# fudan-zvg/PARTNER

Hardware: AMD Instinct MI355X
Metric: frames/sec polar voxelize+PFN+BEV+head, 30k-pt sweep (whole job) (higher is better)
Workload: dtype f32

## Files before the change

include/partner_hip.h:

```cpp
#ifndef PARTNER_HIP_H
#define PARTNER_HIP_H

#include <stddef.h>
#include <stdint.h>

#ifdef __cplusplus
extern "C" {
#endif

#define PN_OK 0
#define PN_ERR_INVALID (-1)
#define PN_ERR_LAUNCH (-2)
#define PN_ERR_WORKSPACE (-3)

#define PN_ACT_NONE 0
#define PN_ACT_RELU 1
#define PN_ACT_TANH 2
#define PN_ACT_GELU 3

typedef void *pn_stream_t;

int pn_version(void);
int pn_last_error(char *buf, size_t buf_len);
int pn_device_count(void);
// ... 472 lines not shown
                               void *workspace, size_t workspace_bytes, pn_stream_t stream);
typedef struct {
  const float *src;
  int32_t pixel_stride;
  int32_t rows;
} pn_row_piece;
int pn_assemble_rows_f32(const pn_row_piece *pieces, int n_out, int out_rows, int w, int c, float *out,
                         int out_pixel_stride, int out_channel_offset, pn_stream_t stream);

int pn_nchw_to_nhwc_f32(const float *in, int b, int c, int h, int w, float *out, pn_stream_t stream);
int pn_nhwc_to_nchw_f32(const float *in, int b, int c, int h, int w, int pixel_stride,
                        int channel_offset, float *out, pn_stream_t stream);
int pn_transpose_hw_f32(const float *in, int b, int h, int w, int c, float *out, pn_stream_t stream);

typedef struct {
  pn_conv_desc desc;
  const float *in;
  const float *packed_w;
  const float *scale;
  const float *shift;
  float *out;
  float *stat_partials;
  int32_t stat_strata;
  int32_t stat_channel_groups;
  const float *stat_gamma;
  const float *stat_beta;
  float stat_eps;
  int32_t stat_affine_strata;
  float *stat_affine;
  float *stat_mean_rstd;
  const float *norm_affine;
  int32_t norm_strata;
  int32_t norm_channels;
} pn_conv_job;
size_t pn_conv_wino_packed_weight_floats(int cout, int cin);
int pn_pack_conv_weight_wino_f32(const float *w_oihw, int cout, int cin, float *packed, pn_stream_t stream);
int pn_pack_conv_dgrad_weight_wino_f32(const float *w_fwd_oihw, int cout_fwd, int cin_fwd, float *packed, pn_stream_t stream);
int pn_conv2d_wino_nhwc_f32(const pn_conv_desc *desc, const float *in, const float *packed_w, const float *scale,
                            const float *shift, float *out, pn_stream_t stream);
size_t pn_conv_wino4_packed_weight_floats(int cout, int cin);
int pn_pack_conv_weight_wino4_f32(const float *w_oihw, int cout, int cin, float *packed, pn_stream_t stream);
int pn_pack_conv_dgrad_weight_wino4_f32(const float *w_fwd_oihw, int cout_fwd, int cin_fwd, float *packed, pn_stream_t stream);
int pn_conv_wino4_tiles(const pn_conv_desc *desc);
int pn_conv2d_wino4_nhwc_f32(const pn_conv_desc *desc, const float *in, const float *packed_w, const float *scale,
                             const float *shift, float *out, pn_stream_t stream);
size_t pn_wino4_planes_floats(int batch, int h, int w, int c);
int pn_wino4_planes_from_nhwc_f32(const float *in, int batch, int h, int w, int c, int in_pixel_stride, int in_channel_offset,
                                  int transpose_hw, float *planes, pn_stream_t stream);
int pn_conv_wino4_chain_supported(const pn_conv_desc *desc);
int pn_conv2d_wino4_chain_f32(const pn_conv_desc *desc, const float *planes_in, const float *packed_w, const float *scale,
                              const float *shift, float *planes_out, float *out_nhwc, pn_stream_t stream);
size_t pn_conv_wino24_packed_weight_floats(int cout, int cin);
int pn_pack_conv_weight_wino24_f32(const float *w_oihw, int cout, int cin, float *packed, pn_stream_t stream);
int pn_conv_wino24_chain_supported(const pn_conv_desc *desc);
int pn_conv2d_wino24_chain_f32(const pn_conv_desc *desc, const float *planes_in, const float *packed_w24, const float *scale,
                               const float *shift, float *planes_out, float *out_nhwc, pn_stream_t stream);

size_t pn_conv_wino44_packed_weight_floats(int cout, int cin);
int pn_pack_conv_weight_wino44_f32(const float *w_oihw, int cout, int cin, float *packed, pn_stream_t stream);
int pn_conv_wino44_chain_supported(const pn_conv_desc *desc);
int pn_conv2d_wino44_chain_f32(const pn_conv_desc *desc, const float *planes_in, const float *packed_w44, const float *scale,
                               const float *shift, float *planes_out, float *out_nhwc, pn_stream_t stream);
typedef struct pn_head_stat_job {
  const float *partials;
  int32_t cout_total;
  int32_t channel_offset;
// ... 121 lines not shown
```

partner_amd/csrc/conv_mfma.hip:

```cpp
#include "pn_common.h"
#include "wino_planes.h"
#include <algorithm>
#include <cstdlib>

namespace {

using f32x16 = __attribute__((ext_vector_type(16))) float;
using f32x4 = __attribute__((ext_vector_type(4))) float;
using bf16x8 = __attribute__((ext_vector_type(8))) __bf16;

enum { DT_F32 = 0, DT_BF16 = 1, DT_BF16_F32OUT = 2 };

__device__ __forceinline__ unsigned short f32_to_bf16_rne(float f) {
  unsigned u = __builtin_bit_cast(unsigned, f);
  u += 0x7fffu + ((u >> 16) & 1u);
  return (unsigned short)(u >> 16);
}

enum { MODE_CONV = 0, MODE_DECONV2 = 1, MODE_STRAT = 2 };

struct ConvArgs {
  const float* in;
  const float* w;
  const float* scale;
// ... 539 lines not shown
          rpix = ((size_t)b * (2 * a.OH) + 2 * oh + (col_d[j] >> 1)) * (2 * a.OW) + 2 * ow + (col_d[j] & 1);
          dst = a.out + rpix * a.out_ps + col_off[j];
        }
        float o;
        if (a.res && a.res_pre_act) {
          o = pn::apply_act(fmaf(acc[i][j][r], sc[j], sh[j]) + a.res[rpix * a.res_ps + col_off[j]], a.act);
        } else {
          o = pn::apply_act(fmaf(acc[i][j][r], sc[j], sh[j]), a.act);
          if (a.res) o += a.res[rpix * a.res_ps + col_off[j]];
        }
        if constexpr (DT == DT_BF16)
          reinterpret_cast<unsigned short*>(a.out)[dst - a.out] = f32_to_bf16_rne(o);
        else
          *dst = o;
      }
    }
  }
}


template <int WM, int WN, int TM, int TN, int DT = DT_F32, bool GATHER = false, bool NORM_IN = false>
__global__ __launch_bounds__(WM* WN * 64) void conv_mfma_kernel(ConvArgs a) {
  constexpr int BN = WN * TN * 32;
  int bid = blockIdx.x;
  if constexpr (!GATHER) {
    const int nmt = a.nmt, q = nmt >> 3, r = nmt & 7, x = bid & 7, idx = bid >> 3;
    bid = (x < r ? x * (q + 1) : r * (q + 1) + (x - r) * q) + idx;
  }
  conv_body<WM, WN, TM, TN, DT, GATHER, NORM_IN>(a, bid, blockIdx.y * BN, blockIdx.z);
}

constexpr int kMaxJobs = 8;
struct MultiArgs {
  int njobs, total;
  int first[kMaxJobs + 1];
  ConvArgs job[kMaxJobs];
};

template <int WM, int WN, int TM, int TN, bool NORM_IN>
__global__ __launch_bounds__(WM* WN * 64) void conv_multi_kernel(MultiArgs m_by_value) {
  constexpr int BN = WN * TN * 32;
  typedef const __attribute__((address_space(4))) int* kptr_t;
  const kptr_t base = (kptr_t)__builtin_amdgcn_kernarg_segment_ptr();
  const int njobs = base[offsetof(MultiArgs, njobs) / 4], nt = base[offsetof(MultiArgs, total) / 4];
  const int bid = blockIdx.x;
  const int q = nt >> 3, r = nt & 7, x = bid & 7, idx = bid >> 3;
  const int t = (x < r ? x * (q + 1) : r * (q + 1) + (x - r) * q) + idx;
  int j = 0;
  for (int k = 1; k < njobs; ++k)
    if (t >= base[offsetof(MultiArgs, first) / 4 + k]) j = k;
  j = __builtin_amdgcn_readfirstlane(j);
  const int local = t - base[offsetof(MultiArgs, first) / 4 + j];
  static_assert(sizeof(ConvArgs) % 4 == 0 && offsetof(MultiArgs, job) % 4 == 0, "job table must be dword aligned");
  constexpr int JW = sizeof(ConvArgs) / 4;
  union { ConvArgs a; int w[JW]; } u;
  const kptr_t src = base + offsetof(MultiArgs, job) / 4 + j * JW;
#pragma unroll
  for (int i = 0; i < JW; ++i) u.w[i] = src[i];
  const ConvArgs& a = u.a;
  const int ntn = (a.ncols + BN - 1) / BN, per_z = a.nmt * ntn;
  const int z = local / per_z, rem = local - z * per_z;
  const int ny = rem / a.nmt, mt = rem - ny * a.nmt;
  conv_body<WM, WN, TM, TN, DT_F32, false, NORM_IN>(a, mt, ny * BN, z);
}


struct FinArgs {
  int njobs, total;
  int first[kMaxJobs + 1];
  int bm, wn;
  ConvArgs job[kMaxJobs];
};

__device__ __forceinline__ void group_geometry(const ConvArgs& a, int& pix_b, int& wsub, int& spr) {
  pix_b = a.OH * a.OWsub;
  wsub = a.OWsub / a.st_S;
  spr = a.st_S > 1 ? wsub / 32 : 1;
}

template <int NT>
__device__ __forceinline__ void fold_allch_group(const ConvArgs& a, const float2* part, int wn_count, int z, int b, int s, double* red,
                                                 double& o1, double& o2) {
  int pix_b, wsub, spr;
  group_geometry(a, pix_b, wsub, spr);
  const int tid = threadIdx.x;
// ... 1046 lines not shown
__global__ void f32_to_bf16_kernel(const float* __restrict__ x, unsigned short* __restrict__ y, size_t n) {
  for (size_t i = blockIdx.x * (size_t)blockDim.x + threadIdx.x; i < n; i += (size_t)gridDim.x * blockDim.x) y[i] = f32_to_bf16_rne(x[i]);
}

__global__ void bf16_to_f32_kernel(const unsigned short* __restrict__ x, float* __restrict__ y, size_t n) {
  for (size_t i = blockIdx.x * (size_t)blockDim.x + threadIdx.x; i < n; i += (size_t)gridDim.x * blockDim.x)
    y[i] = __builtin_bit_cast(float, (unsigned)x[i] << 16);
}

template <int WM, int WN, int TM, int TN, bool NORM_IN>
int launch_multi(MultiArgs& m, size_t extra_smem, hipStream_t st) {
  constexpr int BM = WM * TM * 32, BN = WN * TN * 32;
  constexpr size_t base = 2 * (size_t)(BM * A_LD + BK * BN) * sizeof(float);
  const size_t smem = base + extra_smem;
  PN_REQUIRE(smem <= 160 * 1024, "conv_multi: the normalisation table does not fit LDS");
  static size_t attr_smem[64] = {0};
  int dev = 0;
  (void)hipGetDevice(&dev);
  if (dev < 0 || dev >= 64 || attr_smem[dev] < smem) {
    (void)hipFuncSetAttribute(reinterpret_cast<const void*>(&conv_multi_kernel<WM, WN, TM, TN, NORM_IN>),
                              hipFuncAttributeMaxDynamicSharedMemorySize, (int)smem);
    if (dev >= 0 && dev < 64) attr_smem[dev] = smem;
  }
  int total = 0;
  for (int j = 0; j < m.njobs; ++j) {
    ConvArgs& a = m.job[j];
    a.nmt = pn::cdiv(a.M, BM);
    const int tiles_z = a.nmt * pn::cdiv(a.ncols, BN);
    m.first[j] = total;
    total += tiles_z * a.zdim;
  }
  m.first[m.njobs] = total;
  m.total = total;
  pn::ProfileSlot ps;
  if (pn::take_profile_slot(ps))
    hipExtLaunchKernelGGL((conv_multi_kernel<WM, WN, TM, TN, NORM_IN>), dim3(total), dim3(WM * WN * 64), smem, st, ps.start, ps.stop, 0, m);
  else
    hipLaunchKernelGGL((conv_multi_kernel<WM, WN, TM, TN, NORM_IN>), dim3(total), dim3(WM * WN * 64), smem, st, m);
  return pn::check_launch("conv_multi_kernel");
}

int tile_bm(int tile) { return tile == 1 ? 128 : 64; }

}

extern "C" {

}

namespace {

template <int K>
__device__ __forceinline__ float quad_bcast(float v) {
  return __builtin_bit_cast(float, __builtin_amdgcn_update_dpp(0, __builtin_bit_cast(int, v), K * 0x55, 0xf, 0xf, true));
}

template <int CIN>
__global__ __launch_bounds__(256) void sparse_conv_c16_kernel(const float* __restrict__ in, unsigned in_bytes, const int32_t* __restrict__ nbr,
                                                              const int32_t* __restrict__ n_out, int cap, int taps, const float* __restrict__ packed_w,
                                                              int quads, int cout_pad, const float* __restrict__ scale, const float* __restrict__ shift,
                                                              int act, const float* __restrict__ residual, float* __restrict__ out) {
  __shared__ __attribute__((aligned(16))) float wl[27 * 256];
  __shared__ int nb_s[64 * 27];
  const int tid = threadIdx.x, q = tid & 3, sl = tid >> 2;
  for (int i = tid; i < taps * 256; i += 256) {
    const int t = i >> 8, ci = (i >> 4) & 15, co = i & 15;
    wl[i] = ci < CIN ? packed_w[(((size_t)t * quads + (ci >> 2)) * cout_pad + co) * 4 + (ci & 3)] : 0.f;
  }
  const int n = min(*n_out, cap);
  const __amdgpu_buffer_rsrc_t rsrc = __builtin_amdgcn_make_buffer_rsrc(const_cast<float*>(in), 0, in_bytes, 0x00020000);
  const f32x4 sc = scale ? *reinterpret_cast<const f32x4*>(scale + 4 * q) : f32x4{1.f, 1.f, 1.f, 1.f};
  const f32x4 sh = shift ? *reinterpret_cast<const f32x4*>(shift + 4 * q) : f32x4{0.f, 0.f, 0.f, 0.f};
  for (int g = blockIdx.x; g * 64 < n; g += gridDim.x) {
    __syncthreads();
    for (int i = tid; i < 64 * taps; i += 256) nb_s[i] = g * 64 + i / taps < n ? nbr[(size_t)g * 64 * taps + i] : -1;
// ... 213 lines not shown
                              pn_stream_t stream) {
  PN_REQUIRE(pn_conv2d_nhwc_planes_supported(d), "conv_planes: not covered (groups 1, cout % 8 == 0, output rows of 4 .. 64 pixels dividing 64, or of 128)");
  PN_REQUIRE(in && packed_w && planes && ((uintptr_t)in & 15) == 0 && ((uintptr_t)packed_w & 15) == 0 && ((uintptr_t)planes & 15) == 0 &&
                 ((uintptr_t)scale & 15) == 0 && ((uintptr_t)shift & 15) == 0, "conv_planes: null or misaligned pointer");
  ConvArgs a;
  int zdim = 1;
  if (int rc = fill_args(d, a, zdim)) return rc;
  a.in = in; a.w = packed_w; a.scale = scale; a.shift = shift;
  a.out = planes; a.out_ps = d->cout; a.out_co = 0;
  a.planes = planes;
  a.plane_floats = (unsigned)((size_t)d->batch * (a.OH + 2) * (a.OW / 4) * 4);
  hipStream_t st = pn::S(stream);
  if (a.OW == 128) {
    const long long t128 = (long long)pn::cdiv(a.M, 128) * pn::cdiv(a.ncols, 128);
    return t128 >= 384 ? launch_conv<2, 2, 2, 2>(a, zdim, st) : launch_conv<4, 2, 1, 1>(a, zdim, st);
  }
  return dispatch_conv(a, zdim, st);
}

size_t pn_conv_stat_partial_floats(const pn_conv_desc* d, int tile) {
  ConvArgs a;
  int zdim = 1;
  if (fill_args(d, a, zdim)) return 0;
  const int bm = tile_bm(tile);
  return (size_t)zdim * pn::cdiv(a.M, bm) * (bm / 32) * a.cout_pad * 2;
}

static int tile_wn(int tile) { return tile == 5 ? 4 : (tile == 4 ? 1 : 2); }

static int job_to_args(const pn_conv_job& jb, int tile, ConvArgs& a, size_t& extra) {
  int zdim = 1;
  if (int rc = fill_args(&jb.desc, a, zdim)) return rc;
  const pn_conv_desc* d = &jb.desc;
  PN_REQUIRE(jb.in && jb.packed_w && jb.out, "conv_multi: null pointer");
  PN_REQUIRE(d->cin % 4 == 0 && d->in_pixel_stride % 4 == 0 && d->in_channel_offset % 4 == 0,
             "conv_multi: cin, input pixel stride and channel offset must be multiples of 4");
  PN_REQUIRE(((uintptr_t)jb.in & 15) == 0 && ((uintptr_t)jb.packed_w & 15) == 0, "conv_multi: pointers must be 16-byte aligned");
  PN_REQUIRE(!d->accumulate, "conv_multi: accumulate is not supported");
  a.in = jb.in; a.w = jb.packed_w; a.scale = jb.scale; a.shift = jb.shift; a.out = jb.out;
  a.zdim = zdim;
  const int bm = tile_bm(tile), bn = tile_wn(tile) * (tile == 1 ? 64 : 32);
  a.nmt = pn::cdiv(a.M, bm);
  a.st_segs_z = a.nmt * (bm / 32);
  if (jb.stat_partials) {
    PN_REQUIRE(a.mode != MODE_DECONV2, "conv_multi: no statistics for the transposed convolution");
    PN_REQUIRE((a.Cout % 4 == 0) && (a.out_ps % 4 == 0) && (a.out_co % 4 == 0) && (((uintptr_t)a.out & 15) == 0),
               "conv_multi: statistics need the vectorised epilogue (channel counts / offsets multiples of 4)");
    PN_REQUIRE(a.mode == MODE_STRAT || zdim == 1, "conv_multi: statistics of grouped convolutions are not supported");
    PN_REQUIRE(a.ncols <= bn, "conv_multi: statistics need the job's columns in one column tile");
    const int S = jb.stat_strata < 1 ? 1 : jb.stat_strata;
    PN_REQUIRE(S == 1 || (a.mode == MODE_CONV && a.OWsub % S == 0 && (a.OWsub / S) % 32 == 0),
               "conv_multi: stat_strata needs a plain convolution whose strata are multiples of 32 columns");
    PN_REQUIRE(a.B == 1 || (a.OH * a.OWsub) % (jb.stat_channel_groups > 1 ? bm : 32) == 0,
               "conv_multi: with batch > 1 a sample must be a whole number of tiles (per-channel statistics) / 32-row segments");
    PN_REQUIRE(jb.stat_channel_groups == 1 || jb.stat_channel_groups == a.ncols, "conv_multi: channel groups must be 1 or the column count");
    const int slots = a.mode == MODE_STRAT ? zdim : S;
    PN_REQUIRE(jb.stat_affine_strata >= slots, "conv_multi: stat_affine_strata too small");
    a.st_part = jb.stat_partials; a.st_S = S; a.st_cg = jb.stat_channel_groups;
    a.st_gamma = jb.stat_gamma; a.st_beta = jb.stat_beta; a.st_eps = jb.stat_eps;
    a.st_ab = jb.stat_affine; a.st_ab_S = jb.stat_affine_strata; a.st_stat = jb.stat_mean_rstd;
  }
  if (jb.norm_affine) {
    PN_REQUIRE(jb.norm_strata >= 1 && a.W % jb.norm_strata == 0 && a.KW <= 3 && a.KH * a.KW <= 16, "conv_multi: bad normalise-on-load geometry");
    PN_REQUIRE(jb.norm_channels >= a.Cin * (d->groups > 1 ? d->groups : 1) && a.B * jb.norm_strata < 1024, "conv_multi: normalisation table too small / too many groups");
    a.ni_ab = jb.norm_affine; a.ni_S = jb.norm_strata; a.ni_C = jb.norm_channels;
    extra = std::max(extra, (size_t)a.B * a.ni_S * a.ni_C * 2 * sizeof(float));
  }
  return PN_OK;
}

int pn_conv2d_multi_f32(const pn_conv_job* jobs, int njobs, int tile, pn_stream_t stream) {
  PN_REQUIRE(jobs && njobs >= 1 && njobs <= kMaxJobs, "conv_multi: 1 .. 8 jobs");
  PN_REQUIRE(tile == 1 || tile == 3 || tile == 4 || tile == 5, "conv_multi: tile must be 1 (128x128), 3 (64x64), 4 (64x32) or 5 (64x128)");
  MultiArgs m;
  memset(&m, 0, sizeof(m));
  m.njobs = njobs;
  bool norm_in = false;
  size_t extra = 0;
  for (int j = 0; j < njobs; ++j) {
    if (int rc = job_to_args(jobs[j], tile, m.job[j], extra)) return rc;
    norm_in = norm_in || m.job[j].ni_ab != nullptr;
  }
  if (norm_in)
    for (int j = 0; j < njobs; ++j) PN_REQUIRE(m.job[j].ni_ab, "conv_multi: normalise-on-load must be given for every job of the launch or for none");
  hipStream_t st = pn::S(stream);
  switch (tile) {
    case 1: PN_REQUIRE(!norm_in, "conv_multi: tile 1 has no normalise-on-load variant"); return launch_multi<2, 2, 2, 2, false>(m, 0, st);
    case 3: return norm_in ? launch_multi<2, 2, 1, 1, true>(m, extra, st) : launch_multi<2, 2, 1, 1, false>(m, 0, st);
    case 4: return norm_in ? launch_multi<2, 1, 1, 1, true>(m, extra, st) : launch_multi<2, 1, 1, 1, false>(m, 0, st);
    default: PN_REQUIRE(!norm_in, "conv_multi: tile 5 has no normalise-on-load variant"); return launch_multi<2, 4, 1, 1, false>(m, 0, st);
  }
}

int pn_conv3x3_tap_sum_f32(const float* g, int ldg, int batch, int h, int w, int cout, const float* scale, const float* shift, int act, float* out,
                           int out_pixel_stride, int out_channel_offset, pn_stream_t stream) {
  PN_REQUIRE(g && out && batch >= 1 && h >= 1 && w >= 1 && cout >= 1 && cout <= 3 && ldg >= 9 * cout, "conv3x3_tap_sum: bad arguments (cout 1 .. 3, ldg >= 9 cout)");
  PN_REQUIRE(out_pixel_stride >= out_channel_offset + cout && out_channel_offset >= 0, "conv3x3_tap_sum: channel slice does not fit the pixel stride");
  PN_REQUIRE((long long)batch * h * w * cout < (1ll << 31), "conv3x3_tap_sum: map too large");
  const int total = batch * h * w * cout;
  hipLaunchKernelGGL(conv_tap_sum_kernel, dim3(pn::cdiv(total, 256)), dim3(256), 0, pn::S(stream), g, ldg, batch, h, w, cout, scale, shift, act, out,
                     out_pixel_stride, out_channel_offset);
  return pn::check_launch("conv_tap_sum_kernel");
}

int pn_conv2d_small_n_multi_f32(const pn_conv_job* jobs, int njobs, pn_stream_t stream) {
  PN_REQUIRE(jobs && njobs >= 1 && njobs <= kMaxJobs, "conv_small_n_multi: 1 .. 8 jobs");
  MultiArgs m;
  memset(&m, 0, sizeof(m));
  m.njobs = njobs;
  int total = 0;
  int order[kMaxJobs], no = 0;
  for (int pass = 0; pass < 2; ++pass)
    for (int j = 0; j < njobs; ++j)
      if ((jobs[j].desc.kh * jobs[j].desc.kw == 9) == (pass == 0)) order[no++] = j;
  for (int jo = 0; jo < njobs; ++jo) {
    const int j = jo;
    ConvArgs& a = m.job[j];
    size_t extra = 0;
    if (int rc = job_to_args(jobs[order[jo]], 3, a, extra)) return rc;
    const int taps = a.KH * a.KW;
    PN_REQUIRE(a.mode == MODE_CONV && a.zdim == 1 && a.ncols <= 12 && a.Cin <= 64 && (taps == 9 || taps == 1) && !jobs[order[jo]].stat_partials,
               "conv_small_n_multi: plain 1x1 / 3x3 convolutions with <= 64 input channels and <= 12 output columns, no statistics");
// ... 110 lines not shown
```

partner_amd/hip.py:

```python
from __future__ import annotations

import ctypes as C
import os
from typing import Optional

import torch

_LIB_PATH = os.path.join(os.path.dirname(os.path.abspath(__file__)), "lib", "libpartner_hip.so")
_lib: Optional[C.CDLL] = None

ACT_NONE, ACT_RELU, ACT_TANH, ACT_GELU = 0, 1, 2, 3


class PartnerHipError(RuntimeError):
    pass


class ConvDesc(C.Structure):

    _fields_ = [(n, C.c_int32) for n in (
        "batch", "in_h", "in_w", "cin", "cout", "groups", "kh", "kw", "stride", "pad_h", "pad_w",
        "in_pixel_stride", "in_channel_offset", "out_pixel_stride", "out_channel_offset", "act", "deconv2x2",
        "range_strata", "pad_h_end", "pad_w_end", "accumulate", "frames_in_flight", "transpose_hw")]


class RowPiece(C.Structure):

    _fields_ = [("src", C.c_void_p), ("pixel_stride", C.c_int32), ("rows", C.c_int32)]


class HeadStatJob(C.Structure):

    _fields_ = [("partials", C.c_void_p), ("cout_total", C.c_int32), ("channel_offset", C.c_int32), ("channels", C.c_int32), ("strata", C.c_int32),
                ("gamma", C.c_void_p), ("beta", C.c_void_p), ("eps", C.c_float), ("table", C.c_void_p)]


class ChainHeadJob(C.Structure):

    _fields_ = [("desc", C.POINTER(ConvDesc)), ("planes_in", C.c_void_p), ("packed_w24", C.c_void_p), ("scale", C.c_void_p), ("shift", C.c_void_p),
                ("planes_out", C.c_void_p), ("out_nhwc", C.c_void_p), ("stat_partials", C.c_void_p)]


class ConvJob(C.Structure):

    _fields_ = [("desc", ConvDesc), ("in_", C.c_void_p), ("packed_w", C.c_void_p), ("scale", C.c_void_p), ("shift", C.c_void_p),
                ("out", C.c_void_p), ("stat_partials", C.c_void_p), ("stat_strata", C.c_int32),
                ("stat_channel_groups", C.c_int32), ("stat_gamma", C.c_void_p), ("stat_beta", C.c_void_p), ("stat_eps", C.c_float),
                ("stat_affine_strata", C.c_int32), ("stat_affine", C.c_void_p), ("stat_mean_rstd", C.c_void_p),
                ("norm_affine", C.c_void_p), ("norm_strata", C.c_int32), ("norm_channels", C.c_int32)]


_P = C.c_void_p
_I = C.c_int
_F = C.c_float
_SZ = C.c_size_t
_U64 = C.c_uint64

SIGNATURES = {
    "pn_version": (_I, []),
    "pn_last_error": (_I, [C.c_char_p, _SZ]),
    "pn_device_count": (_I, []),
    "pn_cart_to_polar_f32": (_I, [_P, _I, _I, _P, _P]),
    "pn_polar_grid_index_f32": (_I, [_P, _I, _I, _P, _I, _P, _P, _P, _P, _P, _P]),
    "pn_keys_from_grid_ind": (_I, [_P, _I, _P, _I, _P, _P]),
    "pn_unique_workspace_bytes": (_SZ, [_U64, _I]),
    "pn_unique_rank_bitmap": (_I, [_P, _I, _P, _U64, _P, _P, _P, _P, _P, _P, _SZ, _P]),
    "pn_unique_keys_ptr": (_P, [_P, _U64, _I]),
    "pn_bucket_workspace_bytes": (_SZ, [_I]),
    "pn_bucket_points": (_I, [_P, _P, _I, _P, _P, _P, _P, _P, _SZ, _P]),
    "pn_voxel_index_fused_state_bytes": (_SZ, [_U64]),
    "pn_voxel_index_fused_f32": (_I, [_P, _I, _I, _P, _I, _P, _P, _P, _P, _P, _P, _P, _P, _SZ, _P, _P, _P, _P, _P]),
    "pn_voxel_index_fused_rows_f32": (_I, [_P, _I, _I, _P, _I, _P, _P, _P, _P, _P, _P, _P, _P, _SZ, _P, _P, _P, _P, _P, _P]),
    "pn_voxel_index_fused_sweeps_f32": (_I, [_P, _I, _I, _P, _I, _P, _P, _F, _P, _P, _P, _P, _P, _P, _P, _P, _SZ, _P, _P, _P, _P, _P, _P]),
    "pn_clear_frame_cells": (_I, [_P, _P, _I, _P, _I, _P, _P, _P]),
    "pn_sort_voxel_runs": (_I, [_P, _P, _I, _P, _P, _P]),
    "pn_hard_voxelize_workspace_bytes": (_SZ, [_U64, _I, _I]),
    "pn_hard_voxelize_f32": (_I, [_P, _I, _I, _I, _P, _P, _I, _I, _P, _P, _P, _P, _P, _SZ, _P]),
    "pn_scatter_mean_f32": (_I, [_P, _I, _I, _P, _P, _P, _I, _P, _P]),
    "pn_hard_voxel_mean_f32": (_I, [_P, _P, _I, _I, _I, _P, _P]),
    "pn_concat_voxel_segments_f32": (_I, [_P, _P, _P, _I, _I, _I, _P, _P, _P, _P]),
    "pn_dynamic_pfn_fwd": (_I, [_P, _I, _P, _P, _P, _I, _P, _P, _P, _I, _P, _I, _F, _F, _F, _F, _P, _P, _P]),
    "pn_pfn_center_table_floats": (_SZ, [_I]),
# ... 283 lines not shown
```

partner_amd/necks.py:

```python
from __future__ import annotations

import logging

import numpy as np
import torch
from torch import nn

from . import hip, ops
from .builder import NECKS
from .nn_utils import PlanCache, Sequential, build_norm_layer, eval_only


@NECKS.register_module
class RPN(nn.Module):
    def __init__(self, layer_nums, ds_layer_strides, ds_num_filters, us_layer_strides, us_num_filters,
                 num_input_features, norm_cfg=None, name="rpn", logger=None, **kwargs):
        super().__init__()
        self._layer_strides = ds_layer_strides
        self._num_filters = ds_num_filters
        self._layer_nums = layer_nums
        self._upsample_strides = us_layer_strides
        self._num_upsample_filters = us_num_filters
        self._num_input_features = num_input_features
        self._norm_cfg = norm_cfg or dict(type="BN", eps=1e-3, momentum=0.01)
# ... 64 lines not shown
                plan["pillar0"] = ops.PillarConvLayer(c0.weight, c0.stride[0], scale=scale, shift=shift, act=ops.ACT_RELU)
        for blk in self.blocks:
            mods = list(blk._modules.values())
            layers = [self._fused(mods[1], mods[2], mods[1].stride[0], 1, dtype=dtype)]
            for k in range(4, len(mods), 3):
                layers.append(self._fused(mods[k], mods[k + 1], 1, 1, dtype=dtype))
            plan["blocks"].append(layers)
        for de in self.deblocks:
            up, bn = de[0], de[1]
            if isinstance(up, nn.ConvTranspose2d):
                if up.stride[0] == 1 and up.kernel_size[0] == 1:
                    w1 = up.weight.detach().permute(1, 0, 2, 3).contiguous()
                    scale, shift = ops.fold_bn(bn.weight, bn.bias, bn.running_mean, bn.running_var, bn.eps, up.bias)
                    plan["deblocks"].append(ops.ConvLayer(w1, stride=1, pad=0, scale=scale, shift=shift, act=ops.ACT_RELU, dtype=dtype))
                    continue
                if up.stride[0] != 2:
                    raise NotImplementedError("RPN deblock: only ConvTranspose2d(k=2, s=2) / (k=1, s=1) have a HIP kernel")
                plan["deblocks"].append(self._fused(up, bn, 1, 0, deconv=True, dtype=dtype))
            else:
                plan["deblocks"].append(self._fused(up, bn, up.stride[0], 0, dtype=dtype))
        return plan

    def forward_nhwc(self, x: torch.Tensor, return_blocks=False, pillars=None):
        eval_only(self, "RPN")
        dtype = getattr(self, "compute_dtype", "f32")
        if dtype == "bf16":
            if not hasattr(self, "_plan_bf16"):
                self._plan_bf16 = PlanCache()
            plan = self._plan_bf16.get(self, lambda: self._build_plan("bf16"))
            x = ops.to_bf16(x)
        else:
            plan = self._plan.get(self, self._build_plan)
        out, off, block_outs = None, 0, []
        self.canvas_read_by_pillars_only = False
        for i, layers in enumerate(plan["blocks"]):
            for k, layer in enumerate(layers):
                p0 = plan.get("pillar0") if (i == 0 and k == 0 and pillars is not None and dtype == "f32") else None
                if p0 is not None and p0.worth_it(pillars, x.shape[0], x.shape[1], x.shape[2]):
                    b0, oh, ow = x.shape[0], (x.shape[1] - 1) // p0.stride + 1, (x.shape[2] - 1) // p0.stride + 1
                    rest = layers[1:]
                    self.canvas_read_by_pillars_only = p0.rows_form(pillars, b0, x.shape[1], x.shape[2])
                    if (rest and all(l.stride == 1 for l in rest) and p0.planes_supported(b0, x.shape[1], x.shape[2])
                            and ops.conv_chain_orientation(rest, b0, oh, ow) is False):
                        canvas = x
                        x = ops.conv_chain(rest, None, shape=(b0, oh, ow), device=x.device, planes_from=lambda buf: p0(canvas, pillars, planes=buf))
                        break
                    x = p0(x, pillars)
                elif (k == 0 and dtype == "f32" and layer.stride > 1 and len(layers) > 1 and all(l.stride == 1 for l in layers[1:])
                      and layer.planes_desc(*x.shape) is not None
                      and ops.conv_chain_orientation(layers[1:], x.shape[0], *layer.out_hw(x.shape[1], x.shape[2])) is False):
                    src, b0 = x, x.shape[0]
                    oh, ow = layer.out_hw(x.shape[1], x.shape[2])
                    x = ops.conv_chain(layers[1:], None, shape=(b0, oh, ow), device=x.device, planes_from=lambda buf, l=layer, s=src: l.to_planes(s, buf))
                    break
                elif k <= 1 and dtype == "f32" and layer.stride == 1 and ops.conv_chain_supported(layers[k:], x.shape[0], x.shape[1], x.shape[2]):
                    x = ops.conv_chain(layers[k:], x)
                    break
                else:
                    x = layer(x)
            block_outs.append(x)
            j = i - self._upsample_start_idx
            if j >= 0:
                de = plan["deblocks"][j]
                if out is None:
                    oh, ow = de.out_hw(x.shape[1], x.shape[2])
                    odt = torch.bfloat16 if (dtype == "bf16" and getattr(self, "bf16_output", False) and not return_blocks) else torch.float32
                    out = torch.empty((x.shape[0], oh, ow, sum(self._num_upsample_filters)), dtype=odt, device=x.device)
                de(x, out=out, out_channel_offset=off)
                off += self._num_upsample_filters[j]
        res = out if out is not None else x
        return (res, block_outs) if return_blocks else res

    def forward(self, x):
        eval_only(self, "RPN")
        hip.require_device(x)
        return ops.as_nchw(self.forward_nhwc(ops.to_nhwc(x)))
```

partner_amd/ops_conv.py:

```python
from __future__ import annotations

import ctypes as C
from dataclasses import dataclass
from typing import Optional, Sequence, Tuple

import torch

from . import hip
from .hip import ACT_NONE, ACT_RELU, ACT_TANH, ConvDesc
from .ops_common import *
from .ops_common import _f32, _workspace
from .routes import R, S
from .ops_index import VoxelIndex



class frames_in_flight:

    def __init__(self, n: int):
        self.n, self.prev = max(1, int(n)), 1

    def __enter__(self):
        self.prev, S.frames_in_flight = S.frames_in_flight, self.n
        return self
# ... 573 lines not shown
            out = torch.empty((b, oh, ow, self.cout), dtype=torch.float32, device=canvas.device)
        cap = (vi.n_cap + 127) // 128 * 128
        ws = _workspace(9 * cap * self.cout * 4, canvas.device)
        hip.call("pn_pillar_conv3x3_tables_f32", canvas.data_ptr(), b, oh, ow, self.cin, ct, 0, tables.data_ptr(), vi.n_cap, self.packed.data_ptr(), self.cout,
                 hip.ptr(self.scale), hip.ptr(self.shift), self.act, out.data_ptr(), out.shape[3], 0, ws.data_ptr(), ws.numel(), hip.stream())
        return out

    def dgrad_features(self, dout: torch.Tensor, vi: "VoxelIndex", tables: torch.Tensor) -> torch.Tensor:
        hip.require_device(dout)
        assert dout.is_contiguous() and dout.shape[3] >= self.cout
        b, oh, ow, ct = dout.shape
        dfeat = torch.empty((max(vi.n_cap, 1), self.cin), dtype=torch.float32, device=dout.device)
        cap = (vi.n_cap + 127) // 128 * 128
        ws = _workspace(9 * cap * self.cin * 4, dout.device)
        hip.call("pn_pillar_conv3x3_dgrad_f32", dout.data_ptr(), b, oh, ow, self.cout, ct, 0, tables.data_ptr(), vi.num_voxels.data_ptr(), vi.n_cap,
                 self.packed_t.data_ptr(), self.cin, dfeat.data_ptr(), ws.data_ptr(), ws.numel(), hip.stream())
        return dfeat

    def wgrad(self, canvas: torch.Tensor, dout: torch.Tensor, vi: "VoxelIndex", tables: torch.Tensor, out: Optional[torch.Tensor] = None,
              accumulate=False) -> torch.Tensor:
        lib = hip.load()
        b, oh, ow, ct = dout.shape
        if out is None:
            out = torch.empty((self.cout, self.cin, 3, 3), dtype=torch.float32, device=dout.device)
        nbytes = lib.pn_pillar_conv_wgrad_workspace_bytes(vi.n_cap, self.cin, self.cout)
        ws = _workspace(nbytes, dout.device)
        hip.call("pn_pillar_conv3x3_wgrad_f32", canvas.data_ptr(), canvas.shape[3], 0, self.cin, dout.data_ptr(), ct, 0, self.cout, tables.data_ptr(), vi.n_cap,
                 b, oh, ow, out.data_ptr(), int(accumulate), ws.data_ptr(), nbytes, hip.stream())
        return out


class ConvJob:

    def __init__(self, layer: "ConvLayer", x: torch.Tensor, out: torch.Tensor, in_channel_offset=0, out_channel_offset=0, stats=None,
                 norm=None):
        assert layer.dtype == "f32" and not layer.deconv2x2
        hip.require_device(x, out)
        assert x.dim() == 4 and x.is_contiguous() and out.is_contiguous() and x.dtype == torch.float32
        self.layer, self.x, self.out, self.in_co, self.out_co, self.stats, self.norm = layer, x, out, in_channel_offset, out_channel_offset, stats, norm
        b, h, w, ct = x.shape
        oh, ow = layer.out_hw(h, w)
        assert out.shape[:3] == (b, oh, ow)
        self.desc = ConvDesc(b, h, w, layer.cin, layer.cout, layer.groups, layer.kh, layer.kw, layer.stride, layer.pad[0], layer.pad[1],
                             ct, in_channel_offset, out.shape[3], out_channel_offset, layer.act, 0, layer.range_strata, 0, 0, 0)
        self.macs = b * oh * ow * layer.groups * layer.cout * layer.cin * layer.kh * layer.kw

    def partial_floats(self, tile: int) -> int:
        return int(hip.load().pn_conv_stat_partial_floats(C.byref(self.desc), tile))



def _job_array(jobs: Sequence[ConvJob]):
    arr = (hip.ConvJob * len(jobs))()
    for k, jb in enumerate(jobs):
        c = arr[k]
        c.desc = jb.desc
        jb.layer._packs.ensure("direct")
        c.in_, c.packed_w, c.out = jb.x.data_ptr(), jb.layer.packed.data_ptr(), jb.out.data_ptr()
        c.scale, c.shift = hip.ptr(jb.layer.scale), hip.ptr(jb.layer.shift)
        if jb.stats is not None:
            st = jb.stats
            c.stat_partials = st["partials"].data_ptr()
            c.stat_strata, c.stat_channel_groups = int(st.get("strata", 1)), int(st["channel_groups"])
            c.stat_gamma, c.stat_beta, c.stat_eps = hip.ptr(st.get("gamma")), hip.ptr(st.get("beta")), float(st["eps"])
            c.stat_affine_strata = int(st["affine_strata"])
            c.stat_affine, c.stat_mean_rstd = hip.ptr(st.get("affine")), hip.ptr(st.get("mean_rstd"))
        if jb.norm is not None:
            tab, strata, channels = jb.norm
            c.norm_affine, c.norm_strata, c.norm_channels = tab.data_ptr(), int(strata), int(channels)
    return arr


def conv_multi(jobs: Sequence[ConvJob], tile: int) -> None:
    arr = _job_array(jobs)
    st = hip.stream()
    prof = S.profiler
    if prof is not None:
        ev = prof.begin(st)
    hip.call("pn_conv2d_multi_f32", arr, len(jobs), int(tile), st)
    if prof is not None:
        j0 = jobs[0]
        prof.end(ev, 2.0 * sum(j.macs for j in jobs), st,
                 tag=f"multi x{len(jobs)} {j0.out.shape[1]}x{j0.out.shape[2]} {sum(j.layer.cin * j.layer.groups for j in jobs)}->{sum(j.layer.out_channels for j in jobs)} k{j0.layer.kh}")


def conv_small_n_multi(jobs: Sequence[ConvJob]) -> None:
    st = hip.stream()
    prof = S.profiler
    if prof is not None:
        ev = prof.begin(st)
    hip.call("pn_conv2d_small_n_multi_f32", _job_array(jobs), len(jobs), st)
    if prof is not None:
        j0 = jobs[0]
        prof.end(ev, 2.0 * sum(j.macs for j in jobs), st,
                 tag=f"small-n x{len(jobs)} {j0.out.shape[1]}x{j0.out.shape[2]} {sum(j.layer.cin * j.layer.groups for j in jobs)}->{sum(j.layer.out_channels for j in jobs)}")


def conv_stats_finalize(jobs: Sequence[ConvJob], tile: int) -> None:
    hip.call("pn_conv_stats_finalize_f32", _job_array(jobs), len(jobs), int(tile), hip.stream())


def conv_stats_apply(producer: ConvJob, tile: int, gamma, beta, act, out: torch.Tensor, out_channel_offset=0, mul=None, add=None,
                     out2: Optional[torch.Tensor] = None, out2_channel_offset=0) -> None:
    hip.require_device(out)
    hip.call("pn_conv_stats_apply_f32", _job_array([producer]), int(tile), hip.ptr(gamma), hip.ptr(beta), int(act), out.data_ptr(), out.shape[3],
             out_channel_offset, hip.ptr(mul), hip.ptr(add), hip.ptr(out2), 0 if out2 is None else out2.shape[3], out2_channel_offset, hip.stream())


def groupnorm_apply(x: torch.Tensor, channel_groups: int, range_strata: int, mean_rstd: torch.Tensor, gamma, beta, act, out: torch.Tensor,
                    out_channel_offset=0, mul=None, add=None, out2: Optional[torch.Tensor] = None, out2_channel_offset=0,
                    channels: Optional[int] = None, channel_offset=0) -> None:
    hip.require_device(x, out, mean_rstd)
    b, h, w, ct = x.shape
    c = ct - channel_offset if channels is None else channels
    hip.call("pn_groupnorm_apply_f32", x.data_ptr(), b, h, w, c, ct, channel_offset, channel_groups, range_strata, mean_rstd.data_ptr(),
             hip.ptr(gamma), hip.ptr(beta), int(act), out.data_ptr(), out.shape[3], out_channel_offset, hip.ptr(mul), hip.ptr(add), hip.ptr(out2),
# ... 47 lines not shown
```

partner_amd/routes.py:

```python
from __future__ import annotations

import os
from contextlib import contextmanager


class Routes:
    def __init__(self):
        self.conv_wino = os.environ.get("PN_CONV_WINO", "1") != "0"
        self.conv_wino_min_tiles = int(os.environ.get("PN_CONV_WINO_MIN_TILES", "256"))
        self.conv_wino4 = os.environ.get("PN_CONV_WINO4", "1") != "0"
        self.conv_wino4_min_tiles = int(os.environ.get("PN_CONV_WINO4_MIN_TILES", "256"))
        self.conv_wino4_dgrad = os.environ.get("PN_CONV_WINO4_DGRAD", "1") != "0"
        self.conv_tapsum = os.environ.get("PN_CONV_TAPSUM", "1") != "0"
        self.conv_chain = os.environ.get("PN_CONV_CHAIN", "1") != "0"
        self.conv_chain2d = os.environ.get("PN_CONV_CHAIN2D", "1") != "0"
        self.conv_chain44 = os.environ.get("PN_CONV_CHAIN44", "1") != "0"
        self.conv_planes = os.environ.get("PN_CONV_PLANES", "1") != "0"
        self.conv_wgrad_wino4 = os.environ.get("PN_CONV_WGRAD_WINO4", "1") != "0"
        self.conv_wgrad_wino4_min_quads = int(os.environ.get("PN_CONV_WGRAD_WINO4_MIN_QUADS", "4096"))
        self.pillar_conv = os.environ.get("PN_PILLAR_CONV", "1") != "0"
        self.pillar_planes = os.environ.get("PN_PILLAR_PLANES", "1") != "0"
        self.pillar_rows = os.environ.get("PN_PILLAR_ROWS", "1") != "0"
        self.pillar_conv_max_fill = float(os.environ.get("PN_PILLAR_CONV_MAX_FILL", "0.35"))
        self.pillar_rows_max_fill = float(os.environ.get("PN_PILLAR_ROWS_MAX_FILL", "1.25"))
        self.fused_sweeps = os.environ.get("PN_FUSED_SWEEPS", "1") != "0"
        self.sample_streams = os.environ.get("PN_SAMPLE_STREAMS", "1") != "0"
        self.pfn_clears_index = os.environ.get("PN_PFN_CLEARS_INDEX", "1") != "0"
        self.linear = os.environ.get("PN_LINEAR", "1") != "0"
        self.ln_fold = os.environ.get("PN_LN_FOLD", "1") != "0"
        self.head_chain = os.environ.get("PN_HEAD_CHAIN", "1") != "0"
        self.sparse_c16 = os.environ.get("PN_SPARSE_C16", "1") != "0"
        self.sparse_row_bits = os.environ.get("PN_SPARSE_ROW_BITS", "1") != "0"
        self.sparse_grouped = os.environ.get("PN_SPARSE_GROUPED", "1") != "0"
        self.sparse_struct_stream = os.environ.get("PN_SPARSE_STRUCT_STREAM", "1") != "0"
        self.train_wgrad_stream = os.environ.get("PN_TRAIN_WGRAD_STREAM", "1") != "0"
        self.train_wino4_max_pixels = int(os.environ.get("PN_TRAIN_WINO4_MAX_PIXELS", "16384"))
        self.train_pillar_conv = os.environ.get("PN_TRAIN_PILLAR_CONV", "1") != "0"
        self.train_prepack = os.environ.get("PN_TRAIN_PREPACK", "1") != "0"
        self.train_chain_max_pixels = int(os.environ.get("PN_TRAIN_CHAIN_MAX_PIXELS", "4096"))
        self.train_strat_expand = os.environ.get("PN_TRAIN_STRAT_EXPAND", "0") != "0"

    @contextmanager
    def override(self, **kw):
        old = {k: getattr(self, k) for k in kw}
        try:
            for k, v in kw.items():
                setattr(self, k, v)
            yield self
        finally:
            for k, v in old.items():
# ... 15 lines not shown
```

Before: 1838.

## Co-launch upsample deconv with next block's strided planes conv in one multi-job kernel

The neck now defers each block's upsample (deblock) convolution and launches it together with the next block's strided first convolution in a single multi-job kernel. The strided conv writes directly into winograd planes for the following chain. A per-job tile-dealing mode handles jobs with different K depths, and a new 128x64 tile variant is added. This is meant to cut launch count and fill the GPU better with two small independent convs, at the cost of more complex scheduling and possible imbalance between unequal jobs.

```diff
diff --git a/include/partner_hip.h b/include/partner_hip.h
--- a/include/partner_hip.h
+++ b/include/partner_hip.h
@@ -528,6 +528,7 @@
   const float *norm_affine;
   int32_t norm_strata;
   int32_t norm_channels;
+  float *planes;
 } pn_conv_job;
 size_t pn_conv_wino_packed_weight_floats(int cout, int cin);
 int pn_pack_conv_weight_wino_f32(const float *w_oihw, int cout, int cin, float *packed, pn_stream_t stream);
diff --git a/partner_amd/csrc/conv_mfma.hip b/partner_amd/csrc/conv_mfma.hip
--- a/partner_amd/csrc/conv_mfma.hip
+++ b/partner_amd/csrc/conv_mfma.hip
@@ -595,7 +595,7 @@
 
 constexpr int kMaxJobs = 8;
 struct MultiArgs {
-  int njobs, total;
+  int njobs, total, per_job;
   int first[kMaxJobs + 1];
   ConvArgs job[kMaxJobs];
 };
@@ -606,14 +606,19 @@
   typedef const __attribute__((address_space(4))) int* kptr_t;
   const kptr_t base = (kptr_t)__builtin_amdgcn_kernarg_segment_ptr();
   const int njobs = base[offsetof(MultiArgs, njobs) / 4], nt = base[offsetof(MultiArgs, total) / 4];
+  const bool per_job = base[offsetof(MultiArgs, per_job) / 4] != 0;
   const int bid = blockIdx.x;
-  const int q = nt >> 3, r = nt & 7, x = bid & 7, idx = bid >> 3;
-  const int t = (x < r ? x * (q + 1) : r * (q + 1) + (x - r) * q) + idx;
+  auto deal = [](int i, int n) {
+    const int q = n >> 3, r = n & 7, x = i & 7, idx = i >> 3;
+    return (x < r ? x * (q + 1) : r * (q + 1) + (x - r) * q) + idx;
+  };
+  const int t = per_job ? bid : deal(bid, nt);
   int j = 0;
   for (int k = 1; k < njobs; ++k)
     if (t >= base[offsetof(MultiArgs, first) / 4 + k]) j = k;
   j = __builtin_amdgcn_readfirstlane(j);
-  const int local = t - base[offsetof(MultiArgs, first) / 4 + j];
+  const int first_j = base[offsetof(MultiArgs, first) / 4 + j];
+  const int local = per_job ? deal(t - first_j, base[offsetof(MultiArgs, first) / 4 + j + 1] - first_j) : t - first_j;
   static_assert(sizeof(ConvArgs) % 4 == 0 && offsetof(MultiArgs, job) % 4 == 0, "job table must be dword aligned");
   constexpr int JW = sizeof(ConvArgs) / 4;
   union { ConvArgs a; int w[JW]; } u;
@@ -1726,6 +1731,11 @@
   }
   m.first[m.njobs] = total;
   m.total = total;
+  m.per_job = 0;
+  for (int j = 1; j < m.njobs; ++j) {
+    const ConvArgs &a = m.job[j], &a0 = m.job[0];
+    if (a.KH * a.KW * a.cin_chunks != a0.KH * a0.KW * a0.cin_chunks) m.per_job = 1;
+  }
   pn::ProfileSlot ps;
   if (pn::take_profile_slot(ps))
     hipExtLaunchKernelGGL((conv_multi_kernel<WM, WN, TM, TN, NORM_IN>), dim3(total), dim3(WM * WN * 64), smem, st, ps.start, ps.stop, 0, m);
@@ -1734,7 +1744,7 @@
   return pn::check_launch("conv_multi_kernel");
 }
 
-int tile_bm(int tile) { return tile == 1 ? 128 : 64; }
+int tile_bm(int tile) { return tile == 1 || tile == 7 ? 128 : 64; }
 
 }
 
@@ -2014,7 +2024,7 @@
   int zdim = 1;
   if (int rc = fill_args(&jb.desc, a, zdim)) return rc;
   const pn_conv_desc* d = &jb.desc;
-  PN_REQUIRE(jb.in && jb.packed_w && jb.out, "conv_multi: null pointer");
+  PN_REQUIRE(jb.in && jb.packed_w && (jb.out || jb.planes), "conv_multi: null pointer");
   PN_REQUIRE(d->cin % 4 == 0 && d->in_pixel_stride % 4 == 0 && d->in_channel_offset % 4 == 0,
              "conv_multi: cin, input pixel stride and channel offset must be multiples of 4");
   PN_REQUIRE(((uintptr_t)jb.in & 15) == 0 && ((uintptr_t)jb.packed_w & 15) == 0, "conv_multi: pointers must be 16-byte aligned");
@@ -2023,6 +2033,16 @@
   a.zdim = zdim;
   const int bm = tile_bm(tile), bn = tile_wn(tile) * (tile == 1 ? 64 : 32);
   a.nmt = pn::cdiv(a.M, bm);
+  if (jb.planes) {
+    PN_REQUIRE(pn_conv2d_nhwc_planes_supported(d), "conv_multi: planes job not covered (groups 1, cout % 8 == 0, output rows of 4 .. 64 pixels dividing 64, or of 128)");
+    PN_REQUIRE(bm % a.OW == 0, "conv_multi: a planes job needs whole map rows in the tile's %d pixels (output rows of %d)", bm, a.OW);
+    PN_REQUIRE(!jb.stat_partials && !jb.norm_affine, "conv_multi: a planes job takes no statistics and no normalise-on-load");
+    PN_REQUIRE(((uintptr_t)jb.planes & 15) == 0 && ((uintptr_t)jb.scale & 15) == 0 && ((uintptr_t)jb.shift & 15) == 0,
+               "conv_multi: planes, scale and shift of a planes job must be 16-byte aligned");
+    a.out = jb.planes; a.out_ps = d->cout; a.out_co = 0;
+    a.planes = jb.planes;
+    a.plane_floats = (unsigned)((size_t)d->batch * (a.OH + 2) * (a.OW / 4) * 4);
+  }
   a.st_segs_z = a.nmt * (bm / 32);
   if (jb.stat_partials) {
     PN_REQUIRE(a.mode != MODE_DECONV2, "conv_multi: no statistics for the transposed convolution");
@@ -2053,7 +2073,7 @@
 
 int pn_conv2d_multi_f32(const pn_conv_job* jobs, int njobs, int tile, pn_stream_t stream) {
   PN_REQUIRE(jobs && njobs >= 1 && njobs <= kMaxJobs, "conv_multi: 1 .. 8 jobs");
-  PN_REQUIRE(tile == 1 || tile == 3 || tile == 4 || tile == 5, "conv_multi: tile must be 1 (128x128), 3 (64x64), 4 (64x32) or 5 (64x128)");
+  PN_REQUIRE(tile == 1 || tile == 3 || tile == 4 || tile == 5 || tile == 7, "conv_multi: tile must be 1 (128x128), 3 (64x64), 4 (64x32), 5 (64x128) or 7 (128x64)");
   MultiArgs m;
   memset(&m, 0, sizeof(m));
   m.njobs = njobs;
@@ -2070,6 +2090,7 @@
     case 1: PN_REQUIRE(!norm_in, "conv_multi: tile 1 has no normalise-on-load variant"); return launch_multi<2, 2, 2, 2, false>(m, 0, st);
     case 3: return norm_in ? launch_multi<2, 2, 1, 1, true>(m, extra, st) : launch_multi<2, 2, 1, 1, false>(m, 0, st);
     case 4: return norm_in ? launch_multi<2, 1, 1, 1, true>(m, extra, st) : launch_multi<2, 1, 1, 1, false>(m, 0, st);
+    case 7: PN_REQUIRE(!norm_in, "conv_multi: tile 7 has no normalise-on-load variant"); return launch_multi<4, 2, 1, 1, false>(m, 0, st);
     default: PN_REQUIRE(!norm_in, "conv_multi: tile 5 has no normalise-on-load variant"); return launch_multi<2, 4, 1, 1, false>(m, 0, st);
   }
 }
diff --git a/partner_amd/hip.py b/partner_amd/hip.py
--- a/partner_amd/hip.py
+++ b/partner_amd/hip.py
@@ -47,7 +47,7 @@
                 ("out", C.c_void_p), ("stat_partials", C.c_void_p), ("stat_strata", C.c_int32),
                 ("stat_channel_groups", C.c_int32), ("stat_gamma", C.c_void_p), ("stat_beta", C.c_void_p), ("stat_eps", C.c_float),
                 ("stat_affine_strata", C.c_int32), ("stat_affine", C.c_void_p), ("stat_mean_rstd", C.c_void_p),
-                ("norm_affine", C.c_void_p), ("norm_strata", C.c_int32), ("norm_channels", C.c_int32)]
+                ("norm_affine", C.c_void_p), ("norm_strata", C.c_int32), ("norm_channels", C.c_int32), ("planes", C.c_void_p)]
 
 
 _P = C.c_void_p
diff --git a/partner_amd/necks.py b/partner_amd/necks.py
--- a/partner_amd/necks.py
+++ b/partner_amd/necks.py
@@ -120,6 +120,13 @@
         else:
             plan = self._plan.get(self, self._build_plan)
         out, off, block_outs = None, 0, []
+
+        def planes_route(layers, x):
+            layer = layers[0]
+            return (dtype == "f32" and layer.stride > 1 and len(layers) > 1 and all(l.stride == 1 for l in layers[1:])
+                    and layer.planes_desc(*x.shape) is not None
+                    and ops.conv_chain_orientation(layers[1:], x.shape[0], *layer.out_hw(x.shape[1], x.shape[2])) is False)
+        deferred = None
         self.canvas_read_by_pillars_only = False
         for i, layers in enumerate(plan["blocks"]):
             for k, layer in enumerate(layers):
@@ -134,12 +141,15 @@
                         x = ops.conv_chain(rest, None, shape=(b0, oh, ow), device=x.device, planes_from=lambda buf: p0(canvas, pillars, planes=buf))
                         break
                     x = p0(x, pillars)
-                elif (k == 0 and dtype == "f32" and layer.stride > 1 and len(layers) > 1 and all(l.stride == 1 for l in layers[1:])
-                      and layer.planes_desc(*x.shape) is not None
-                      and ops.conv_chain_orientation(layers[1:], x.shape[0], *layer.out_hw(x.shape[1], x.shape[2])) is False):
+                elif k == 0 and planes_route(layers, x):
                     src, b0 = x, x.shape[0]
                     oh, ow = layer.out_hw(x.shape[1], x.shape[2])
-                    x = ops.conv_chain(layers[1:], None, shape=(b0, oh, ow), device=x.device, planes_from=lambda buf, l=layer, s=src: l.to_planes(s, buf))
+                    if deferred is not None:
+                        (de, de_off, tile), deferred = deferred, None
+                        producer = lambda buf, l=layer, s=src: ops.conv_colaunch(l, de, s, buf, out, de_off, tile)
+                    else:
+                        producer = lambda buf, l=layer, s=src: l.to_planes(s, buf)
+                    x = ops.conv_chain(layers[1:], None, shape=(b0, oh, ow), device=x.device, planes_from=producer)
                     break
                 elif k <= 1 and dtype == "f32" and layer.stride == 1 and ops.conv_chain_supported(layers[k:], x.shape[0], x.shape[1], x.shape[2]):
                     x = ops.conv_chain(layers[k:], x)
@@ -154,8 +164,14 @@
                     oh, ow = de.out_hw(x.shape[1], x.shape[2])
                     odt = torch.bfloat16 if (dtype == "bf16" and getattr(self, "bf16_output", False) and not return_blocks) else torch.float32
                     out = torch.empty((x.shape[0], oh, ow, sum(self._num_upsample_filters)), dtype=odt, device=x.device)
-                de(x, out=out, out_channel_offset=off)
+                nxt = plan["blocks"][i + 1] if i + 1 < len(plan["blocks"]) else None
+                tile = ops.conv_colaunch_tile(nxt[0], de, *x.shape) if nxt is not None and out.dtype == torch.float32 and planes_route(nxt, x) else None
+                if tile is not None:
+                    deferred = (de, off, tile)
+                else:
+                    de(x, out=out, out_channel_offset=off)
                 off += self._num_upsample_filters[j]
+        assert deferred is None
         res = out if out is not None else x
         return (res, block_outs) if return_blocks else res
 
diff --git a/partner_amd/ops_conv.py b/partner_amd/ops_conv.py
--- a/partner_amd/ops_conv.py
+++ b/partner_amd/ops_conv.py
@@ -629,17 +629,25 @@
 
 class ConvJob:
 
-    def __init__(self, layer: "ConvLayer", x: torch.Tensor, out: torch.Tensor, in_channel_offset=0, out_channel_offset=0, stats=None,
-                 norm=None):
+    def __init__(self, layer: "ConvLayer", x: torch.Tensor, out: Optional[torch.Tensor], in_channel_offset=0, out_channel_offset=0, stats=None,
+                 norm=None, planes: Optional[torch.Tensor] = None):
         assert layer.dtype == "f32" and not layer.deconv2x2
-        hip.require_device(x, out)
-        assert x.dim() == 4 and x.is_contiguous() and out.is_contiguous() and x.dtype == torch.float32
+        hip.require_device(x, out, planes)
+        assert x.dim() == 4 and x.is_contiguous() and x.dtype == torch.float32
         self.layer, self.x, self.out, self.in_co, self.out_co, self.stats, self.norm = layer, x, out, in_channel_offset, out_channel_offset, stats, norm
+        self.planes = planes
         b, h, w, ct = x.shape
         oh, ow = layer.out_hw(h, w)
-        assert out.shape[:3] == (b, oh, ow)
+        self.out_hw = (oh, ow)
+        if planes is not None:
+            assert out is None and stats is None and norm is None
+            assert planes.numel() >= hip.load().pn_wino4_planes_floats(b, oh, ow, layer.cout)
+            out_ps, out_channel_offset = layer.cout, 0
+        else:
+            assert out.is_contiguous() and out.shape[:3] == (b, oh, ow)
+            out_ps = out.shape[3]
         self.desc = ConvDesc(b, h, w, layer.cin, layer.cout, layer.groups, layer.kh, layer.kw, layer.stride, layer.pad[0], layer.pad[1],
-                             ct, in_channel_offset, out.shape[3], out_channel_offset, layer.act, 0, layer.range_strata, 0, 0, 0)
+                             ct, in_channel_offset, out_ps, out_channel_offset, layer.act, 0, layer.range_strata, 0, 0, 0)
         self.macs = b * oh * ow * layer.groups * layer.cout * layer.cin * layer.kh * layer.kw
 
     def partial_floats(self, tile: int) -> int:
@@ -653,7 +661,7 @@
         c = arr[k]
         c.desc = jb.desc
         jb.layer._packs.ensure("direct")
-        c.in_, c.packed_w, c.out = jb.x.data_ptr(), jb.layer.packed.data_ptr(), jb.out.data_ptr()
+        c.in_, c.packed_w, c.out, c.planes = jb.x.data_ptr(), jb.layer.packed.data_ptr(), hip.ptr(jb.out), hip.ptr(jb.planes)
         c.scale, c.shift = hip.ptr(jb.layer.scale), hip.ptr(jb.layer.shift)
         if jb.stats is not None:
             st = jb.stats
@@ -668,7 +676,7 @@
     return arr
 
 
-def conv_multi(jobs: Sequence[ConvJob], tile: int) -> None:
+def conv_multi(jobs: Sequence[ConvJob], tile: int, tag: Optional[str] = None) -> None:
     arr = _job_array(jobs)
     st = hip.stream()
     prof = S.profiler
@@ -678,7 +686,26 @@
     if prof is not None:
         j0 = jobs[0]
         prof.end(ev, 2.0 * sum(j.macs for j in jobs), st,
-                 tag=f"multi x{len(jobs)} {j0.out.shape[1]}x{j0.out.shape[2]} {sum(j.layer.cin * j.layer.groups for j in jobs)}->{sum(j.layer.out_channels for j in jobs)} k{j0.layer.kh}")
+                 tag=tag or f"multi x{len(jobs)} {j0.out_hw[0]}x{j0.out_hw[1]} {sum(j.layer.cin * j.layer.groups for j in jobs)}->{sum(j.layer.out_channels for j in jobs)} k{j0.layer.kh}")
+
+
+def conv_colaunch_tile(layer: "ConvLayer", de: "ConvLayer", b: int, h: int, w: int, ct: int) -> Optional[int]:
+    if not R.conv_colaunch or S.frames_in_flight > 1 or layer.planes_desc(b, h, w, ct) is None:
+        return None
+    if (de.dtype != "f32" or de.deconv2x2 or de.range_strata > 1 or de.groups != 1 or de.cin % 4 or de.cout <= 8
+            or de.wino_packed is not None or de.tap_packed is not None):
+        return None
+    ow = layer.out_hw(h, w)[1]
+    return 7 if ow == 128 else 3
+
+
+def conv_colaunch(layer: "ConvLayer", de: "ConvLayer", x: torch.Tensor, planes: torch.Tensor, out: torch.Tensor, out_channel_offset: int,
+                  tile: int) -> None:
+    b, h, w, _ = x.shape
+    ja, jb = ConvJob(layer, x, None, planes=planes), ConvJob(de, x, out, out_channel_offset=out_channel_offset)
+    jobs = sorted((ja, jb), key=lambda j: -j.layer.kh * j.layer.kw * j.layer.cin)
+    (oh, ow), (dh, dw) = ja.out_hw, jb.out_hw
+    conv_multi(jobs, tile, tag=f"{oh}x{ow} {layer.cin}->{layer.cout} k{layer.kh} -> planes + {dh}x{dw} {de.cin}->{de.cout} k{de.kh}")
 
 
 def conv_small_n_multi(jobs: Sequence[ConvJob]) -> None:
diff --git a/partner_amd/routes.py b/partner_amd/routes.py
--- a/partner_amd/routes.py
+++ b/partner_amd/routes.py
@@ -16,6 +16,7 @@
         self.conv_chain2d = os.environ.get("PN_CONV_CHAIN2D", "1") != "0"
         self.conv_chain44 = os.environ.get("PN_CONV_CHAIN44", "1") != "0"
         self.conv_planes = os.environ.get("PN_CONV_PLANES", "1") != "0"
+        self.conv_colaunch = os.environ.get("PN_CONV_COLAUNCH", "1") != "0"
         self.conv_wgrad_wino4 = os.environ.get("PN_CONV_WGRAD_WINO4", "1") != "0"
         self.conv_wgrad_wino4_min_quads = int(os.environ.get("PN_CONV_WGRAD_WINO4_MIN_QUADS", "4096"))
         self.pillar_conv = os.environ.get("PN_PILLAR_CONV", "1") != "0"
```

New measurement: 1827. About the same (-0.6%).
